# apapiu/transformer_latent_diffusion

Hardware: AMD Instinct MI355X
Metric: images/sec (256px, 35-step CFG sampling), denoiser only (higher is better)
Workload: dtype bf16; 1 GPU; C1: 100M-param denoiser (d=768, L=12), 32x32x4 latents, 35 steps + CFG 6, DPM-Solver++(2M), 64 images/GPU (model batch 128); images_per_gpu=64, global_batch=64, n_iter=35, parallelism=single GPU

## Files before the change

### transformer_latent_diffusion_amd/_lib.py

```python
from __future__ import annotations

import ctypes as C
import os

_HERE = os.path.dirname(os.path.abspath(__file__))
LIB_PATH = os.environ.get("TLD_LIB", os.path.join(_HERE, "libtld_hip.so"))

DTYPE_F32, DTYPE_BF16, DTYPE_F16 = 0, 1, 2

KERNEL_CLASSES = ("gemm_qkv", "gemm_up", "gemm_down", "attention", "cross_row", "dwconv_gelu", "layernorm",
                  "embed", "tail", "update", "conditioning")

ABI_SYMBOLS = (
    "tld_engine_create", "tld_engine_load_tensor", "tld_engine_finalize_weights", "tld_denoiser_forward",
    "tld_sample", "tld_sample_from", "tld_engine_set_gemm_dtype", "tld_engine_set_low_latency", "tld_debug_gemm_splitk", "tld_debug_quant_mx8", "tld_debug_quant_mx8_host", "tld_debug_gemm_mx8",
    "tld_engine_set_debug", "tld_engine_read_stage", "tld_engine_stage_shape", "tld_engine_set_debug_step", "tld_engine_debug_paths", "tld_debug_gemm_bf16", "tld_debug_gemm_bench", "tld_debug_gemm_plan", "tld_debug_gemm_epilogue",
    "tld_engine_set_profile", "tld_engine_profile_reserve", "tld_engine_get_profile", "tld_engine_weight_bytes", "tld_engine_destroy",
    "tld_vae_create", "tld_vae_load_tensor", "tld_vae_finalize_weights", "tld_vae_decode", "tld_vae_set_debug",
    "tld_vae_read_stage", "tld_vae_set_profile", "tld_vae_get_profile", "tld_debug_conv3x3", "tld_vae_weight_bytes",
    "tld_vae_destroy",
    "tld_vae_enc_create", "tld_vae_enc_load_tensor", "tld_vae_enc_finalize_weights", "tld_vae_enc_encode", "tld_vae_enc_set_debug",
    "tld_vae_enc_read_stage", "tld_vae_enc_set_profile", "tld_vae_enc_get_profile", "tld_vae_enc_weight_bytes", "tld_vae_enc_destroy",
    "tld_debug_conv3x3_s2",
    "tld_clip_create", "tld_clip_load_tensor", "tld_clip_finalize_weights", "tld_clip_encode_text", "tld_clip_read_buffer", "tld_clip_weight_bytes",
    "tld_clip_destroy",
    "tld_train_create", "tld_train_param_count", "tld_train_tensor_count", "tld_train_param_layout", "tld_train_set_angular_speeds", "tld_train_bind",
# ... 170 lines not shown
```

### transformer_latent_diffusion_amd/csrc/tld_common.h

```cpp
#pragma once
#include <hip/hip_runtime.h>
#include <atomic>
#include <mutex>
#include <stdint.h>
#include "tld_gemm_plan.h"

namespace tld {

typedef __attribute__((ext_vector_type(8))) __bf16 bf16x8;
typedef __attribute__((ext_vector_type(4))) __bf16 bf16x4;
typedef __attribute__((ext_vector_type(2))) __bf16 bf16x2;
typedef __attribute__((ext_vector_type(16))) float f32x16;
typedef __attribute__((ext_vector_type(4))) float f32x4;
typedef __attribute__((ext_vector_type(4))) unsigned u32x4;
typedef __attribute__((ext_vector_type(8))) int i32x8;
typedef __attribute__((ext_vector_type(2))) float f32x2;

constexpr int kWave = 64;
constexpr int kHeadDim = 64;
constexpr float kLnEps = 1e-5f;

template <int CTRL>
__device__ __forceinline__ float dpp_add(float v) {
    const int s = __builtin_amdgcn_update_dpp(0, __float_as_int(v), CTRL, 0xf, 0xf, true);
// ... 314 lines not shown
};
void launch_tail(const TailParams& p, hipStream_t s);

struct UpdateParams {
    const float* x0_2b;
    float* x_t;
    float* x0_prev;
    float* x0_out;
    float* trace_x0; float* trace_xt;
    float g, a, b, c, c1, c2, sharp, bright;
    int final_step;
    int batch, img, chan_stride, C;
};
void launch_update(const UpdateParams& p, hipStream_t s);

struct UpdateFromParams {
    UpdateParams u;
    const float* noise;
    const float* z0;
    const float* mask;
    float s_next;
};
void launch_update_from(const UpdateFromParams& p, hipStream_t s);
void launch_start_mix(const float* noise, const float* z0, float s0, float* x_t, int n, hipStream_t s);

void launch_linear_f32(const float* in, int ldi, const float* W, const float* b, float* out, int ldo,
                       int T, int K, int N, int act, hipStream_t s);
void launch_sinusoid(const float* sigma, const float* angular, float* out, int T, int half, hipStream_t s);
void launch_layernorm_f32(const float* x, const float* g, const float* b, float* out, int M, int d,
                          hipStream_t s);
// ... 12 lines not shown
```

### transformer_latent_diffusion_amd/csrc/tld_engine.hip

```cpp
#include "../../include/tld_hip.h"
#include "tld_common.h"

#include <cmath>
#include <cstdarg>
#include <cstdio>
#include <cstring>
#include <cstdlib>
#include <map>
#include <string>
#include <vector>

using namespace tld;

namespace {

thread_local char g_err[512] = "";

int fail(int code, const char* fmt, ...) {
    va_list ap;
    va_start(ap, fmt);
    vsnprintf(g_err, sizeof(g_err), fmt, ap);
    va_end(ap);
    return code;
}
// ... 50 lines not shown
    float *up_c1 = nullptr, *up_b1 = nullptr;
    float *n1_w = nullptr, *n1_b = nullptr, *n2_w = nullptr, *n2_b = nullptr, *n3_w = nullptr, *n3_b = nullptr;
    float *kv_w = nullptr, *q_w = nullptr;
};

enum { ST_F32 = 0, ST_BF16 = 1, ST_U8 = 2, ST_MX8S = 3, ST_MX8W = 4 };
inline size_t st_bytes(int dtype) { return dtype == ST_F32 ? 4 : dtype == ST_BF16 ? 2 : 1; }
enum { UNPACK_NONE = 0, UNPACK_QKV_ROWS = 1 };
struct DbgStage {
    void* ptr = nullptr; const void* aux = nullptr; int dtype = ST_F32; int64_t shape[4] = {1, 1, 1, 1};
    bool owned = false; size_t cap = 0; bool live = false;
    int64_t outer_stride = 0; int unpack = UNPACK_NONE;
};

enum KClass { KC_GEMM_QKV = 0, KC_GEMM_UP, KC_GEMM_DOWN, KC_ATTN, KC_CROSS, KC_DWCONV, KC_LN, KC_EMBED,
              KC_TAIL, KC_UPDATE, KC_COND, KC_COUNT };

}

struct tld_engine {
    tld_config cfg{};
    int d = 0, L = 0, H = 0, ntok = 0, grid = 0, pd = 0, hid = 0, img = 0, ne = 0, text = 0;
    bool finalized = false;
    bool fuse_dwconv = true;
    bool fp8 = false;
    bool fp8_fused = true;
    uint8_t *a8 = nullptr, *as8 = nullptr;
    std::map<std::string, HostTensor> host;
    std::vector<void*> allocs;
    int64_t weight_bytes = 0;

// ... 3 lines not shown
          *plin_b = nullptr, *pln2_w = nullptr, *pln2_b = nullptr, *pos = nullptr, *out_w = nullptr,
          *out_b = nullptr;
    bf16* out_w_hl = nullptr;
    bf16* plin_w_hl = nullptr;
    std::vector<Layer> layers;
    const float **tab_kv_w = nullptr, **tab_q_w = nullptr, **tab_n2_w = nullptr, **tab_n2_b = nullptr;

    resid_t* x = nullptr;
    resid_t* x_half = nullptr;
    bool share_l0 = true;
    bool fold_ln1 = true;
    bool low_latency = false;
    float* splitk = nullptr;
    int ll_split = 0;
    bool fuse_qkv_attn = true;
    float2* ln_stats = nullptr;
    bool fold_ln3 = true;
    float2* row_stats = nullptr;
    bf16 *xn = nullptr, *qk = nullptr, *vt = nullptr, *att = nullptr, *hid1 = nullptr, *hid2 = nullptr;
    uint32_t* seam = nullptr;
    float *io_x = nullptr, *io_sigma = nullptr, *io_label = nullptr, *io_out = nullptr;
    float *xt = nullptr, *x0_prev = nullptr, *x0_cfg = nullptr;
    int* rows_dev = nullptr;
    int64_t rows_cap = 0;
    void* stage_host = nullptr;
    size_t stage_cap = 0;
    hipEvent_t stage_ev = nullptr;

    int cond_cap = 0;
    float *c_sigma = nullptr, *c_sin = nullptr, *c_h1 = nullptr, *c_pre = nullptr, *c_y = nullptr,
// ... 250 lines not shown
                     (size_t)e->cond_cap * e->H * d, e->c_bwq, (size_t)e->cond_cap * e->H, T, e->H, d, e->L, s);
    return TLD_OK;
}

void cond_noise_rows(tld_engine* e, int Tn, hipStream_t s) {
    launch_sinusoid(e->c_sigma, e->angular, e->c_sin, Tn, e->ne / 2, s);
    launch_linear_f32(e->c_sin, e->ne, e->ff1_w, e->ff1_b, e->c_h1, e->d, Tn, e->ne, e->d, 1, s);
    launch_linear_f32(e->c_h1, e->d, e->ff3_w, e->ff3_b, e->c_pre, e->d, Tn, e->d, e->d, 0, s);
}

void cond_label_rows(tld_engine* e, int row0, int Tl, hipStream_t s) {
    launch_linear_f32(e->c_label, e->text, e->label_w, e->label_b, e->c_pre + (size_t)row0 * e->d, e->d, Tl,
                      e->text, e->d, 0, s);
}

int run_body(tld_engine* e, const float* x_src, int src_batch, int batch, const int* noise_row,
             const int* label_row, float* out, hipStream_t s, bool share_l0 = false) {
    const int d = e->d, M = batch * e->ntok;
    share_l0 = share_l0 && e->share_l0 && batch == 2 * src_batch;
    if (int rc = debug_poison(e, s)) return rc;
    const int b0 = share_l0 ? src_batch : batch;
    resid_t* xe = share_l0 ? e->x_half : e->x;
    const bool fold1 = e->fold_ln1;
    const int ln_slots = gemm_resid_stat_slots(d);
    {
        ProfScope ps(e, KC_EMBED, s);
        EmbedParams ep{};
        ep.x = x_src; ep.conv_w = e->conv_w; ep.conv_b = e->conv_b; ep.ln1_w = e->pln1_w; ep.ln1_b = e->pln1_b;
        ep.lin_wt = e->plin_wt; ep.lin_w_hl = e->plin_w_hl; ep.lin_b = e->plin_b; ep.ln2_w = e->pln2_w; ep.ln2_b = e->pln2_b; ep.pos = e->pos;
        ep.tok = xe; ep.stats_out = fold1 ? e->ln_stats : nullptr; ep.batch = b0; ep.src_batch = src_batch; ep.C = e->cfg.n_channels;
        ep.S = e->cfg.image_size; ep.p = e->cfg.patch_size; ep.grid = e->grid; ep.pd = e->pd; ep.d = d;
        ep.ntok = e->ntok;
        launch_embed(ep, s);
    }
    const int rdt = sizeof(resid_t) == 2 ? ST_BF16 : ST_F32;
    SNAP("tokens0", xe, rdt, s, (int64_t)b0 * e->ntok, d);
    for (int l = 0; l < e->L; ++l) {
        const Layer& Ly = e->layers[l];
        const bool half = share_l0 && l == 0;
        const int bl = half ? b0 : batch, Ml = bl * e->ntok;
        const bool fuse8 = e->fp8 && e->fp8_fused;
        SNAP(blk_name(l, "x_in"), half ? xe : e->x, rdt, s, Ml, d);
        if (fold1) SNAP(blk_name(l, "ln1"), e->ln_stats, ST_F32, s, Ml, kLnSlots, 2);
        if (!fold1) {
            ProfScope ps(e, KC_LN, s);
            if (fuse8 && layernorm_mx8_supported(d)) launch_layernorm_mx8(half ? xe : e->x, Ly.n1_w, Ly.n1_b, e->a8, e->as8, Ml, d, s);
            else { launch_layernorm_bf16(half ? xe : e->x, Ly.n1_w, Ly.n1_b, e->xn, Ml, d, s); SNAP(blk_name(l, "xn1"), e->xn, ST_BF16, s, Ml, d); }
        }
// ... 110 lines not shown
            ProfScope ps(e, KC_GEMM_DOWN, s);
            GemmParams g{};
            g.A = e->hid2; g.lda = e->hid; g.W = Ly.down_w; g.ldw = e->hid; g.M = M; g.N = d; g.K = e->hid;
            g.bias = Ly.down_b; g.resid = e->x; g.ldr = d;
            g.stats_out = (fold1 && l + 1 < e->L) ? e->ln_stats : nullptr;
            if (e->fp8) {
                if (!(fuse8 && e->grid > 16)) launch_quant_mx8(e->hid2, e->a8, e->as8, M, e->hid, s);
                SNAP(blk_name(l, "a8_down.q"), e->a8, ST_U8, s, M, e->hid); SNAP(blk_name(l, "a8_down.s"), e->as8, ST_MX8S, s, M, e->hid / 32);
                g.f8 = 1; g.A = reinterpret_cast<const bf16*>(e->a8); g.W = reinterpret_cast<const bf16*>(Ly.down_w8);
                g.a_scale = e->as8; g.w_scale = Ly.down_s8;
            }
            launch_gemm(g, EPI_BIAS_RESID, s);
        }
        SNAP(blk_name(l, "mlp"), e->x, rdt, s, M, d);
    }
    {
        ProfScope ps(e, KC_TAIL, s);
        TailParams tp{};
        tp.tok = e->x; tp.w = e->out_w; tp.w_hl = e->out_w_hl; tp.b = e->out_b; tp.out = out; tp.batch = batch;
        tp.C = e->cfg.n_channels; tp.S = e->cfg.image_size; tp.p = e->cfg.patch_size; tp.grid = e->grid;
        tp.pd = e->pd; tp.d = d; tp.ntok = e->ntok;
        launch_tail(tp, s);
    }
    SNAP("out", out, ST_F32, s, batch, e->img);
    HIP_TRY(hipGetLastError());
    return TLD_OK;
}

int sample_prepare(tld_engine* e, const void* labels, const float* coeffs, int n_levels, int batch, hipStream_t s, const int** label_row_out) {
    if (!e->finalized) return fail(TLD_ERR_STATE, "weights not finalized");
    if (batch <= 0 || 2 * batch > e->cfg.max_batch)
        return fail(TLD_ERR_INVALID, "sampler batch %d needs max_batch >= %d (have %d)", batch, 2 * batch, e->cfg.max_batch);
    if (n_levels < 2) return fail(TLD_ERR_INVALID, "need at least two noise levels");
    const int B = batch, B2 = 2 * batch, T = n_levels + B + 1;
    if (int rc = ensure_cond_capacity(e, T)) return rc;
    if (int rc = ensure_rows_capacity(e, (int64_t)(n_levels + 1) * B2)) return rc;

    const size_t n_rows = (size_t)(n_levels + 1) * B2;
    if (int rc = debug_begin(e, T, n_levels, s)) return rc;
// ... 22 lines not shown

UpdateParams update_params(tld_engine* e, const float* coeffs, int n_levels, int i, float class_guidance, float sharp_f, float bright_f,
                           void* out_latent, int B, void* trace_x0, void* trace_xt) {
    const bool final_step = (i == n_levels - 1);
    const size_t tot = (size_t)B * e->img;
    UpdateParams up{};
    const float* c = coeffs + (size_t)i * 6;
    up.x0_2b = e->io_out; up.x_t = e->xt; up.x0_prev = e->x0_prev;
    up.x0_out = final_step ? static_cast<float*>(out_latent) : e->x0_cfg;
    up.trace_x0 = (!final_step && trace_x0) ? static_cast<float*>(trace_x0) + (size_t)i * tot : nullptr;
    up.trace_xt = (!final_step && trace_xt) ? static_cast<float*>(trace_xt) + (size_t)i * tot : nullptr;
    up.g = class_guidance; up.a = c[1]; up.b = c[2]; up.c = c[3]; up.c1 = c[4]; up.c2 = c[5];
    up.sharp = sharp_f; up.bright = bright_f; up.final_step = final_step ? 1 : 0;
    up.batch = B; up.img = e->img; up.chan_stride = e->cfg.image_size * e->cfg.image_size; up.C = e->cfg.n_channels;
    return up;
}

int step_begin(tld_engine* e, int i, int B, hipStream_t s) {
    e->dbg_keep = e->debug && (e->dbg_step < 0 || e->dbg_step == i);
    SNAP("step.x_t", e->xt, ST_F32, s, B, e->img); SNAP("step.x0_prev", e->x0_prev, ST_F32, s, B, e->img);
    return TLD_OK;
}
int step_end(tld_engine* e, const UpdateParams& up, int B, hipStream_t s) {
    SNAP("step.out", e->io_out, ST_F32, s, 2 * B, e->img); SNAP("step.x0", up.x0_out, ST_F32, s, B, e->img);
    if (!up.final_step) SNAP("step.x_next", e->xt, ST_F32, s, B, e->img);
    e->dbg_keep = false;
    return TLD_OK;
}

}
// ... 43 lines not shown
    hipDeviceProp_t prop;
    HIP_TRY(hipGetDeviceProperties(&prop, c->device_id));
    if (strncmp(prop.gcnArchName, "gfx950", 6) != 0)
        return fail(TLD_ERR_INVALID, "device %d is %s; this engine is built for gfx950 only", c->device_id, prop.gcnArchName);
    tld_engine* e = new tld_engine();
    e->cfg = *c;
    e->d = c->embed_dim; e->L = c->n_layers; e->H = c->embed_dim / 64; e->grid = grid; e->ntok = ntok;
    e->pd = pd; e->hid = c->mlp_multiplier * c->embed_dim; e->img = c->n_channels * c->image_size * c->image_size;
    e->ne = c->noise_embed_dims; e->text = c->text_emb_size;
    e->layers.resize(e->L);
    if (const char* fd = getenv("TLD_FUSE_DWCONV")) e->fuse_dwconv = atoi(fd) != 0;
    if (const char* sl = getenv("TLD_SHARE_L0")) e->share_l0 = atoi(sl) != 0;
    if (const char* f8 = getenv("TLD_FP8_FUSED")) e->fp8_fused = atoi(f8) != 0;
    if (const char* fl = getenv("TLD_FOLD_LN3")) e->fold_ln3 = atoi(fl) != 0;
    if (const char* fl = getenv("TLD_FOLD_LN1")) e->fold_ln1 = atoi(fl) != 0;
#ifndef TLD_RESID_BF16
    e->fold_ln3 = false;
    e->fold_ln1 = false;
#endif
    e->fold_ln1 = e->fold_ln1 && gemm_resid_stat_slots(e->d) > 0 && (3 * e->d) % 256 == 0;
    e->fold_ln3 = e->fold_ln3 && e->hid % 256 == 0 && cross_row_supports_ln3_stats(e->d);
    if (const char* fq = getenv("TLD_FUSE_QKV_ATTN")) e->fuse_qkv_attn = atoi(fq) != 0;
    e->fuse_qkv_attn = e->fuse_qkv_attn && e->fold_ln1 && ntok == 256 && e->d % 128 == 0;
    *out = e;
    return TLD_OK;
}

int tld_engine_load_tensor(tld_engine* e, const char* key, const void* host_ptr, const int64_t* shape,
                           int32_t ndim, int32_t dtype) {
    if (!e || !key || (!host_ptr && ndim > 0)) return fail(TLD_ERR_INVALID, "null argument");
// ... 416 lines not shown
int tld_sample(tld_engine* e, const void* x_T, const void* labels, const float* coeffs, int32_t n_levels,
               float class_guidance, float sharp_f, float bright_f, void* out_latent, int32_t batch,
               void* trace_x0, void* trace_xt, void* hip_stream) {
    if (!e || !x_T || !labels || !coeffs || !out_latent) return fail(TLD_ERR_INVALID, "null argument");
    DeviceGuard dg(e->cfg.device_id);
    hipStream_t s = static_cast<hipStream_t>(hip_stream);
    const int* label_row = nullptr;
    PathScope paths(e);
    if (int rc = sample_prepare(e, labels, coeffs, n_levels, batch, s, &label_row)) return rc;
    const int B = batch, B2 = 2 * batch;

    const size_t tot = (size_t)B * e->img;
    HIP_TRY(hipMemcpyAsync(e->xt, x_T, tot * sizeof(float), hipMemcpyDeviceToDevice, s));
    HIP_TRY(hipMemsetAsync(e->x0_prev, 0, tot * sizeof(float), s));

    for (int i = 0; i < n_levels; ++i) {
        if (int rc = step_begin(e, i, B, s)) return rc;
        if (int rc = run_body(e, e->xt, B, B2, e->rows_dev + (size_t)i * B2, label_row, e->io_out, s, true)) return rc;
        const UpdateParams up = update_params(e, coeffs, n_levels, i, class_guidance, sharp_f, bright_f, out_latent, B, trace_x0, trace_xt);
        {
            ProfScope ps(e, KC_UPDATE, s);
            launch_update(up, s);
        }
        if (int rc = step_end(e, up, B, s)) return rc;
    }
    HIP_TRY(hipGetLastError());
    return TLD_OK;
}

int tld_sample_from(tld_engine* e, const void* noise, const void* init_latent, const void* mask, float start_mix, const void* labels,
                    const float* coeffs, int32_t n_levels, float class_guidance, float sharp_f, float bright_f, void* out_latent,
// ... 1 lines not shown
    if (!e || !noise || !labels || !coeffs || !out_latent) return fail(TLD_ERR_INVALID, "null argument");
    if (!(start_mix > 0.0f && start_mix <= 1.0f)) return fail(TLD_ERR_INVALID, "start_mix %g outside (0, 1]", (double)start_mix);
    if (!init_latent && (mask || start_mix < 1.0f)) return fail(TLD_ERR_INVALID, "init_latent is required with a mask or with start_mix < 1");
    DeviceGuard dg(e->cfg.device_id);
    hipStream_t s = static_cast<hipStream_t>(hip_stream);
    const int* label_row = nullptr;
    PathScope paths(e);
    if (int rc = sample_prepare(e, labels, coeffs, n_levels, batch, s, &label_row)) return rc;
    const int B = batch, B2 = 2 * batch;

    const size_t tot = (size_t)B * e->img;
    if (start_mix == 1.0f) HIP_TRY(hipMemcpyAsync(e->xt, noise, tot * sizeof(float), hipMemcpyDeviceToDevice, s));
    else launch_start_mix(static_cast<const float*>(noise), static_cast<const float*>(init_latent), start_mix, e->xt, (int)tot, s);
    HIP_TRY(hipMemsetAsync(e->x0_prev, 0, tot * sizeof(float), s));

    for (int i = 0; i < n_levels; ++i) {
        if (int rc = step_begin(e, i, B, s)) return rc;
        if (int rc = run_body(e, e->xt, B, B2, e->rows_dev + (size_t)i * B2, label_row, e->io_out, s, true)) return rc;
        UpdateFromParams uf{};
        uf.u = update_params(e, coeffs, n_levels, i, class_guidance, sharp_f, bright_f, out_latent, B, trace_x0, trace_xt);
        uf.noise = static_cast<const float*>(noise); uf.z0 = static_cast<const float*>(init_latent); uf.mask = static_cast<const float*>(mask);
        uf.s_next = (i + 1 < n_levels) ? coeffs[(size_t)(i + 1) * 6 + 0] : 0.0f;
        {
            ProfScope ps(e, KC_UPDATE, s);
            launch_update_from(uf, s);
        }
        if (int rc = step_end(e, uf.u, B, s)) return rc;
    }
    HIP_TRY(hipGetLastError());
    return TLD_OK;
}
// ... 309 lines not shown
```

### transformer_latent_diffusion_amd/csrc/tld_rows.hip

```cpp
#include "tld_common.h"
#include <cstdlib>

namespace tld {

namespace {


template <int NJ, bool HALF>
__global__ __launch_bounds__(256) void embed_kernel(EmbedParams p) {
    extern __shared__ __attribute__((aligned(16))) char smem[];
    constexpr int d = NJ * 128 - (HALF ? 64 : 0);
    float* wt = reinterpret_cast<float*>(smem);
    float* cwt = wt + p.pd * d;
    for (int i = threadIdx.x; i < p.pd * d / 4; i += 256)
        reinterpret_cast<float4*>(wt)[i] = reinterpret_cast<const float4*>(p.lin_wt)[i];
    for (int i = threadIdx.x; i < p.pd * p.C * p.p * p.p; i += 256) {
        const int o = i / (p.C * p.p * p.p), k = i - o * (p.C * p.p * p.p);
        cwt[k * p.pd + o] = p.conv_w[i];
    }
    __syncthreads();
    const int lane = threadIdx.x & 63;
    const int wid = __builtin_amdgcn_readfirstlane(threadIdx.x >> 6);
    const bool live_last = !HALF || lane < 32;
    auto live = [&](int j) { return j + 1 < NJ || live_last; };
// ... 645 lines not shown
            const int u = uv / p.p, vv = uv - u * p.p;
#pragma unroll
            for (int u2 = 0; u2 < 2; ++u2) {
                const int r = row + u2;
                if (r < total) {
                    const int b = r / p.ntok, t = r - b * p.ntok;
                    const int ti = t / p.grid, tj = t - ti * p.grid;
                    p.out[(((size_t)b * p.C + c) * p.S + (ti * p.p + u)) * p.S + (tj * p.p + vv)] = mine[u2];
                }
            }
        }
    }
}

#ifdef TLD_RESID_BF16
template <int TPW>
__global__ __launch_bounds__(256) void embed_mfma_kernel(EmbedParams p, const bf16* __restrict__ wl_hl) {
    extern __shared__ __attribute__((aligned(16))) char smem[];
    constexpr int d = TPW * 128, PD = 16, PP = 144;
    float* cw = reinterpret_cast<float*>(smem);
    float* red = cw + PD * PD;
    float* vec = red + 4 * 4 * 32;
    char* patch = reinterpret_cast<char*>(vec + 3 * d);
    const int lane = threadIdx.x & 63;
    const int wid = __builtin_amdgcn_readfirstlane(threadIdx.x >> 6);
    const int l31 = lane & 31, hi = lane >> 5;
    const int total = p.batch * p.ntok;
    const int grow = blockIdx.x * 32 + l31;
    const int row = grow < total ? grow : total - 1;
    const int b = row / p.ntok, tk = row - b * p.ntok;
    const int ti = tk / p.grid, tj = tk - ti * p.grid;
    float xin[PD];
    {
        const int pp = p.p * p.p;
        const float* xb = p.x + (size_t)(b % p.src_batch) * p.C * p.S * p.S;
#pragma unroll
        for (int k = 0; k < PD; ++k) {
            const int c = k / pp, uv = k - c * pp, u = uv / p.p, v = uv - u * p.p;
            xin[k] = xb[((size_t)c * p.S + (ti * p.p + u)) * p.S + (tj * p.p + v)];
        }
    }
    bf16x8 whf[TPW], wlf[TPW];
#pragma unroll
    for (int t = 0; t < TPW; ++t) {
        const int f = 32 * (wid * TPW + t) + l31;
        whf[t] = *reinterpret_cast<const bf16x8*>(wl_hl + (size_t)f * PD + hi * 8);
        wlf[t] = *reinterpret_cast<const bf16x8*>(wl_hl + ((size_t)d + f) * PD + hi * 8);
    }
    if (threadIdx.x < PD * PD) cw[threadIdx.x] = p.conv_w[threadIdx.x];
    for (int i = threadIdx.x; i < 3 * d / 4; i += 256) {
        const int which = i / (d / 4), j = i - which * (d / 4);
        const float* src = which == 0 ? p.lin_b : (which == 1 ? p.ln2_w : p.ln2_b);
        reinterpret_cast<float4*>(vec)[i] = reinterpret_cast<const float4*>(src)[j];
    }
    __syncthreads();
    float pv[8];
// ... 106 lines not shown
        }
        __builtin_amdgcn_fence(__ATOMIC_ACQUIRE, "wavefront");
    }
    if (p.stats_out) {
        ssum = pair_sum(ssum); ssq = pair_sum(ssq);
        if (!hi) { red[256 + wid * 32 + l31] = ssum; red[384 + wid * 32 + l31] = ssq; }
        __syncthreads();
        if (wid == 0 && !hi && grow < total) {
            const float a = (red[256 + l31] + red[288 + l31]) + (red[320 + l31] + red[352 + l31]);
            const float a2 = (red[384 + l31] + red[416 + l31]) + (red[448 + l31] + red[480 + l31]);
            *reinterpret_cast<float4*>(p.stats_out + (size_t)grow * kLnSlots) = make_float4(a, a2, 0.f, 0.f);
        }
    }
}

template <int NT>
__global__ __launch_bounds__(256) void tail_mfma_kernel(TailParams p, const bf16* __restrict__ whl) {
    extern __shared__ __attribute__((aligned(16))) char smem[];
    const int d = p.d, PITCH = d * 2, pdp = NT * 16;
    char* wh = smem;
    char* wl = smem + pdp * PITCH;
    const int chunks = d >> 3;
    for (int i = threadIdx.x; i < 2 * pdp * chunks; i += 256) {
        const int plane = i / (pdp * chunks), rem = i - plane * pdp * chunks;
        const int r = rem / chunks, c = rem - r * chunks;
        u32x4 v = {0u, 0u, 0u, 0u};
        if (r < p.pd) v = *reinterpret_cast<const u32x4*>(whl + ((size_t)plane * p.pd + r) * d + c * 8);
        *reinterpret_cast<u32x4*>((plane ? wl : wh) + r * PITCH + ((c ^ (r & 15)) << 4)) = v;
    }
    __syncthreads();
    const int lane = threadIdx.x & 63, wid = threadIdx.x >> 6;
    const int tok = lane & 15, kq = lane >> 4;
    const int total = p.batch * p.ntok;
    const int row0 = (blockIdx.x * 4 + wid) * 16;
    if (row0 >= total) return;
    const int row = row0 + tok < total ? row0 + tok : total - 1;
    const bf16* xrow = p.tok + (size_t)row * d + kq * 8;
    f32x4 acc[NT];
#pragma unroll
    for (int t = 0; t < NT; ++t) acc[t] = f32x4{0.f, 0.f, 0.f, 0.f};
    const int nkb = d >> 5;
    constexpr int PF = 8;
    bf16x8 xf[PF];
#pragma unroll
    for (int i = 0; i < PF; ++i) xf[i] = *reinterpret_cast<const bf16x8*>(xrow + (i < nkb ? i : 0) * 32);
    for (int kb0 = 0; kb0 < nkb; kb0 += PF) {
#pragma unroll
        for (int i = 0; i < PF; ++i) {
            const int kb = kb0 + i;
            if (kb >= nkb) break;
            const bf16x8 xb = xf[i];
            if (kb + PF < nkb) xf[i] = *reinterpret_cast<const bf16x8*>(xrow + (kb + PF) * 32);
            const int chunk = 4 * kb + kq;
#pragma unroll
            for (int t = 0; t < NT; ++t) {
                const int r = t * 16 + tok;
                const int off = r * PITCH + ((chunk ^ (r & 15)) << 4);
                acc[t] = __builtin_amdgcn_mfma_f32_16x16x32_bf16(*reinterpret_cast<const bf16x8*>(wh + off), xb, acc[t], 0, 0, 0);
                acc[t] = __builtin_amdgcn_mfma_f32_16x16x32_bf16(*reinterpret_cast<const bf16x8*>(wl + off), xb, acc[t], 0, 0, 0);
            }
        }
    }
    if (row0 + tok >= total) return;
    const int b = row / p.ntok, tk = row - b * p.ntok;
    const int ti = tk / p.grid, tj = tk - ti * p.grid;
    const int pp = p.p * p.p;
#pragma unroll
    for (int t = 0; t < NT; ++t)
#pragma unroll
        for (int r = 0; r < 4; ++r) {
            const int f = t * 16 + 4 * kq + r;
            if (f < p.pd) {
                const int c = f / pp, uv = f - c * pp;
                const int u = uv / p.p, vv = uv - u * p.p;
                p.out[(((size_t)b * p.C + c) * p.S + (ti * p.p + u)) * p.S + (tj * p.p + vv)] = acc[t][r] + p.b[f];
            }
        }
// ... 82 lines not shown

template <int V>
__global__ __launch_bounds__(256) void start_mix_kernel(const float* __restrict__ noise, const float* __restrict__ z0, float s0,
                                                        float* __restrict__ x_t, int n) {
#pragma clang fp contract(off)
    const int i = (blockIdx.x * 256 + threadIdx.x) * V;
    if (i >= n) return;
    if constexpr (V == 4) {
        const float4 e = *reinterpret_cast<const float4*>(noise + i), z = *reinterpret_cast<const float4*>(z0 + i);
        const float t = 1.0f - s0;
        *reinterpret_cast<float4*>(x_t + i) = make_float4(s0 * e.x + t * z.x, s0 * e.y + t * z.y, s0 * e.z + t * z.z, s0 * e.w + t * z.w);
    } else {
        x_t[i] = s0 * noise[i] + (1.0f - s0) * z0[i];
    }
}

constexpr int DW_CB = 64;
__global__ __launch_bounds__(256) void dwconv_gelu_kernel(const bf16* __restrict__ in, bf16* __restrict__ out,
                                                          const float* __restrict__ w9c,
                                                          const float* __restrict__ bias, int batch,
                                                          int g, int C) {
    extern __shared__ __attribute__((aligned(16))) char smem[];
    const int nchunk = C / DW_CB;
    const int b = blockIdx.x / nchunk, cc = blockIdx.x - b * nchunk;
    const int ntok = g * g;
    const bf16* src = in + (size_t)b * ntok * C + cc * DW_CB;
    for (int idx = threadIdx.x; idx < ntok * 8; idx += 256) {
        const int t = idx >> 3, q = idx & 7;
        *reinterpret_cast<uint4*>(smem + t * 128 + q * 16) =
            *reinterpret_cast<const uint4*>(src + (size_t)t * C + q * 8);
// ... 187 lines not shown
    do {                                                                                             \
        if ((dd) % 128) TLD_DISPATCH_NJ_(((dd) + 127) / 128, true, __VA_ARGS__) else TLD_DISPATCH_NJ_((dd) / 128, false, __VA_ARGS__)  \
    } while (0)

#define TLD_LDS_OPT_IN(KERNEL, bytes)                                                                \
    do {                                                                                             \
        static PerDeviceMax optin;                                                                   \
        if ((bytes) > 64 * 1024)                                                                     \
            optin.run((bytes), [&] { hipFuncSetAttribute(reinterpret_cast<const void*>(KERNEL), hipFuncAttributeMaxDynamicSharedMemorySize, (bytes)); }); \
    } while (0)

void launch_embed(const EmbedParams& p, hipStream_t s) {
#ifdef TLD_RESID_BF16
    if (p.lin_w_hl && p.pd == 16 && p.C * p.p * p.p == 16 && p.d % 256 == 0 && p.d <= 1024) {
        const int rows = p.batch * p.ntok;
        const int lds = 16 * 16 * 4 + 4 * 4 * 32 * 4 + 3 * p.d * 4 + 4 * 32 * 144;
        dim3 grid((unsigned)((rows + 31) / 32));
#define TLD_EM(TPW) do { TLD_LDS_OPT_IN((embed_mfma_kernel<TPW>), lds); hipLaunchKernelGGL((embed_mfma_kernel<TPW>), grid, dim3(256), lds, s, p, p.lin_w_hl); } while (0)
        note_path(EP_EMBED_MFMA + p.d / 256 - 1);
        if (p.d == 256) TLD_EM(2); else if (p.d == 512) TLD_EM(4); else if (p.d == 768) TLD_EM(6); else TLD_EM(8);
#undef TLD_EM
        return;
    }
#endif
    const int rows = p.batch * p.ntok;
    const int lds = (p.pd * p.d + p.pd * p.C * p.p * p.p) * (int)sizeof(float);
    note_path(EP_EMBED_PLAIN);
    TLD_DISPATCH_D(p.d, { TLD_LDS_OPT_IN((embed_kernel<NJ, HALF>), lds); hipLaunchKernelGGL((embed_kernel<NJ, HALF>), dim3((rows + 31) / 32), dim3(256), lds, s, p); });
}

void launch_layernorm_bf16(const resid_t* x, const float* g, const float* b, bf16* out, int M, int d,
// ... 110 lines not shown
#undef TLD_TM
        return;
    }
#endif
    const int rpb = 64;
    const int rows = p.batch * p.ntok;
    const int lds = p.pd * p.d * (int)sizeof(float);
    note_path(EP_TAIL_PLAIN);
    TLD_DISPATCH_D(p.d, { TLD_LDS_OPT_IN((tail_kernel<NJ, HALF>), lds); hipLaunchKernelGGL((tail_kernel<NJ, HALF>), dim3((rows + rpb - 1) / rpb), dim3(256), lds, s, p, rpb); });
}

void launch_update(const UpdateParams& p, hipStream_t s) {
    const int n = p.batch * p.img;
    note_path(EP_UPDATE);
    hipLaunchKernelGGL(update_kernel, dim3((n + 255) / 256), dim3(256), 0, s, p);
}

namespace {
bool aligned16(const void* a) { return (reinterpret_cast<uintptr_t>(a) & 15) == 0; }
}

void launch_update_from(const UpdateFromParams& q, hipStream_t s) {
    const UpdateParams& p = q.u;
    const int n = p.batch * p.img;
    const bool vec = p.img % 4 == 0 && p.chan_stride % 4 == 0 && aligned16(p.x0_2b) && aligned16(p.x_t) && aligned16(p.x0_prev) && aligned16(p.x0_out) &&
                     aligned16(p.trace_x0) && aligned16(p.trace_xt) && aligned16(q.noise) && aligned16(q.z0) && aligned16(q.mask);
    const int threads = vec ? n / 4 : n;
    const dim3 grid((threads + 255) / 256), block(256);
    note_path(q.mask ? EP_UPDATE_FROM_MASK : EP_UPDATE_FROM);
    if (q.mask) {
// ... 242 lines not shown
```

Baseline: 295.3 images/s.

## Fuse tail projection, solver update and next-step embed into one boundary kernel

Adds a step_boundary kernel that, between denoiser steps, does the output projection for both CFG streams, applies the DPM-Solver update, and immediately re-embeds the new latent for the next step. The whole boundary runs per 32-token tile in LDS, replacing three launches and their global round-trips. Also drops the separate step_begin path when fused. The path only runs when share_l0 is on, with no mask, debug, profiling or fp8. It risks numerical differences from the reordered solver arithmetic and higher LDS use per block.

```diff
diff --git a/transformer_latent_diffusion_amd/_lib.py b/transformer_latent_diffusion_amd/_lib.py
--- a/transformer_latent_diffusion_amd/_lib.py
+++ b/transformer_latent_diffusion_amd/_lib.py
@@ -9,7 +9,7 @@
 DTYPE_F32, DTYPE_BF16, DTYPE_F16 = 0, 1, 2
 
 KERNEL_CLASSES = ("gemm_qkv", "gemm_up", "gemm_down", "attention", "cross_row", "dwconv_gelu", "layernorm",
-                  "embed", "tail", "update", "conditioning")
+                  "embed", "tail", "update", "conditioning", "boundary")
 
 ABI_SYMBOLS = (
     "tld_engine_create", "tld_engine_load_tensor", "tld_engine_finalize_weights", "tld_denoiser_forward",
diff --git a/transformer_latent_diffusion_amd/csrc/tld_common.h b/transformer_latent_diffusion_amd/csrc/tld_common.h
--- a/transformer_latent_diffusion_amd/csrc/tld_common.h
+++ b/transformer_latent_diffusion_amd/csrc/tld_common.h
@@ -352,6 +352,10 @@
 };
 void launch_update(const UpdateParams& p, hipStream_t s);
 
+struct BoundaryParams { TailParams t; UpdateParams u; EmbedParams e; };
+bool step_boundary_supported(int d, int pd, int C, int p);
+void launch_step_boundary(const BoundaryParams& q, hipStream_t s);
+
 struct UpdateFromParams {
     UpdateParams u;
     const float* noise;
diff --git a/transformer_latent_diffusion_amd/csrc/tld_engine.hip b/transformer_latent_diffusion_amd/csrc/tld_engine.hip
--- a/transformer_latent_diffusion_amd/csrc/tld_engine.hip
+++ b/transformer_latent_diffusion_amd/csrc/tld_engine.hip
@@ -88,7 +88,7 @@
 };
 
 enum KClass { KC_GEMM_QKV = 0, KC_GEMM_UP, KC_GEMM_DOWN, KC_ATTN, KC_CROSS, KC_DWCONV, KC_LN, KC_EMBED,
-              KC_TAIL, KC_UPDATE, KC_COND, KC_COUNT };
+              KC_TAIL, KC_UPDATE, KC_COND, KC_BOUNDARY, KC_COUNT };
 
 }
 
@@ -122,6 +122,7 @@
     float* splitk = nullptr;
     int ll_split = 0;
     bool fuse_qkv_attn = true;
+    bool fuse_boundary = true;
     float2* ln_stats = nullptr;
     bool fold_ln3 = true;
     float2* row_stats = nullptr;
@@ -402,8 +403,27 @@
                       e->text, e->d, 0, s);
 }
 
+EmbedParams embed_params(const tld_engine* e, const float* x_src, int src_batch, int batch, resid_t* tok) {
+    EmbedParams ep{};
+    ep.x = x_src; ep.conv_w = e->conv_w; ep.conv_b = e->conv_b; ep.ln1_w = e->pln1_w; ep.ln1_b = e->pln1_b;
+    ep.lin_wt = e->plin_wt; ep.lin_w_hl = e->plin_w_hl; ep.lin_b = e->plin_b; ep.ln2_w = e->pln2_w; ep.ln2_b = e->pln2_b; ep.pos = e->pos;
+    ep.tok = tok; ep.stats_out = e->fold_ln1 ? e->ln_stats : nullptr; ep.batch = batch; ep.src_batch = src_batch; ep.C = e->cfg.n_channels;
+    ep.S = e->cfg.image_size; ep.p = e->cfg.patch_size; ep.grid = e->grid; ep.pd = e->pd; ep.d = e->d;
+    ep.ntok = e->ntok;
+    return ep;
+}
+TailParams tail_params(const tld_engine* e, float* out, int batch) {
+    TailParams tp{};
+    tp.tok = e->x; tp.w = e->out_w; tp.w_hl = e->out_w_hl; tp.b = e->out_b; tp.out = out; tp.batch = batch;
+    tp.C = e->cfg.n_channels; tp.S = e->cfg.image_size; tp.p = e->cfg.patch_size; tp.grid = e->grid;
+    tp.pd = e->pd; tp.d = e->d; tp.ntok = e->ntok;
+    return tp;
+}
+
+enum { BODY_EMBED = 1, BODY_TAIL = 2, BODY_ALL = 3 };
+
 int run_body(tld_engine* e, const float* x_src, int src_batch, int batch, const int* noise_row,
-             const int* label_row, float* out, hipStream_t s, bool share_l0 = false) {
+             const int* label_row, float* out, hipStream_t s, bool share_l0 = false, int parts = BODY_ALL) {
     const int d = e->d, M = batch * e->ntok;
     share_l0 = share_l0 && e->share_l0 && batch == 2 * src_batch;
     if (int rc = debug_poison(e, s)) return rc;
@@ -411,15 +431,9 @@
     resid_t* xe = share_l0 ? e->x_half : e->x;
     const bool fold1 = e->fold_ln1;
     const int ln_slots = gemm_resid_stat_slots(d);
-    {
+    if (parts & BODY_EMBED) {
         ProfScope ps(e, KC_EMBED, s);
-        EmbedParams ep{};
-        ep.x = x_src; ep.conv_w = e->conv_w; ep.conv_b = e->conv_b; ep.ln1_w = e->pln1_w; ep.ln1_b = e->pln1_b;
-        ep.lin_wt = e->plin_wt; ep.lin_w_hl = e->plin_w_hl; ep.lin_b = e->plin_b; ep.ln2_w = e->pln2_w; ep.ln2_b = e->pln2_b; ep.pos = e->pos;
-        ep.tok = xe; ep.stats_out = fold1 ? e->ln_stats : nullptr; ep.batch = b0; ep.src_batch = src_batch; ep.C = e->cfg.n_channels;
-        ep.S = e->cfg.image_size; ep.p = e->cfg.patch_size; ep.grid = e->grid; ep.pd = e->pd; ep.d = d;
-        ep.ntok = e->ntok;
-        launch_embed(ep, s);
+        launch_embed(embed_params(e, x_src, src_batch, b0, xe), s);
     }
     const int rdt = sizeof(resid_t) == 2 ? ST_BF16 : ST_F32;
     SNAP("tokens0", xe, rdt, s, (int64_t)b0 * e->ntok, d);
@@ -560,15 +574,13 @@
         }
         SNAP(blk_name(l, "mlp"), e->x, rdt, s, M, d);
     }
-    {
-        ProfScope ps(e, KC_TAIL, s);
-        TailParams tp{};
-        tp.tok = e->x; tp.w = e->out_w; tp.w_hl = e->out_w_hl; tp.b = e->out_b; tp.out = out; tp.batch = batch;
-        tp.C = e->cfg.n_channels; tp.S = e->cfg.image_size; tp.p = e->cfg.patch_size; tp.grid = e->grid;
-        tp.pd = e->pd; tp.d = d; tp.ntok = e->ntok;
-        launch_tail(tp, s);
-    }
-    SNAP("out", out, ST_F32, s, batch, e->img);
+    if (parts & BODY_TAIL) {
+        {
+            ProfScope ps(e, KC_TAIL, s);
+            launch_tail(tail_params(e, out, batch), s);
+        }
+        SNAP("out", out, ST_F32, s, batch, e->img);
+    }
     HIP_TRY(hipGetLastError());
     return TLD_OK;
 }
@@ -621,6 +633,28 @@
     up.sharp = sharp_f; up.bright = bright_f; up.final_step = final_step ? 1 : 0;
     up.batch = B; up.img = e->img; up.chan_stride = e->cfg.image_size * e->cfg.image_size; up.C = e->cfg.n_channels;
     return up;
+}
+
+bool boundary_fused(const tld_engine* e, bool masked) {
+    const uint32_t replaced = (1u << KC_EMBED) | (1u << KC_TAIL) | (1u << KC_UPDATE);
+    return e->fuse_boundary && e->share_l0 && !masked && !e->debug && !(e->prof_mask & replaced) && !e->fp8 && e->out_w_hl && e->plin_w_hl &&
+           step_boundary_supported(e->d, e->pd, e->cfg.n_channels, e->cfg.patch_size);
+}
+
+int fused_step(tld_engine* e, const UpdateParams& up, int i, int B, const int* noise_row, const int* label_row, hipStream_t s) {
+    const int parts = (i == 0 ? BODY_EMBED : 0) | (up.final_step ? BODY_TAIL : 0);
+    if (int rc = run_body(e, e->xt, B, 2 * B, noise_row, label_row, e->io_out, s, true, parts)) return rc;
+    if (up.final_step) {
+        ProfScope ps(e, KC_UPDATE, s);
+        launch_update(up, s);
+    } else {
+        ProfScope ps(e, KC_BOUNDARY, s);
+        BoundaryParams bp{};
+        bp.t = tail_params(e, nullptr, 2 * B); bp.u = up; bp.e = embed_params(e, nullptr, B, B, e->x_half);
+        launch_step_boundary(bp, s);
+    }
+    HIP_TRY(hipGetLastError());
+    return TLD_OK;
 }
 
 int step_begin(tld_engine* e, int i, int B, hipStream_t s) {
@@ -694,6 +728,7 @@
     if (const char* f8 = getenv("TLD_FP8_FUSED")) e->fp8_fused = atoi(f8) != 0;
     if (const char* fl = getenv("TLD_FOLD_LN3")) e->fold_ln3 = atoi(fl) != 0;
     if (const char* fl = getenv("TLD_FOLD_LN1")) e->fold_ln1 = atoi(fl) != 0;
+    if (const char* fb = getenv("TLD_FUSE_BOUNDARY")) e->fuse_boundary = atoi(fb) != 0;
 #ifndef TLD_RESID_BF16
     e->fold_ln3 = false;
     e->fold_ln1 = false;
@@ -1140,7 +1175,13 @@
     HIP_TRY(hipMemcpyAsync(e->xt, x_T, tot * sizeof(float), hipMemcpyDeviceToDevice, s));
     HIP_TRY(hipMemsetAsync(e->x0_prev, 0, tot * sizeof(float), s));
 
+    const bool fused = boundary_fused(e, false);
     for (int i = 0; i < n_levels; ++i) {
+        if (fused) {
+            const UpdateParams up = update_params(e, coeffs, n_levels, i, class_guidance, sharp_f, bright_f, out_latent, B, trace_x0, trace_xt);
+            if (int rc = fused_step(e, up, i, B, e->rows_dev + (size_t)i * B2, label_row, s)) return rc;
+            continue;
+        }
         if (int rc = step_begin(e, i, B, s)) return rc;
         if (int rc = run_body(e, e->xt, B, B2, e->rows_dev + (size_t)i * B2, label_row, e->io_out, s, true)) return rc;
         const UpdateParams up = update_params(e, coeffs, n_levels, i, class_guidance, sharp_f, bright_f, out_latent, B, trace_x0, trace_xt);
@@ -1172,7 +1213,13 @@
     else launch_start_mix(static_cast<const float*>(noise), static_cast<const float*>(init_latent), start_mix, e->xt, (int)tot, s);
     HIP_TRY(hipMemsetAsync(e->x0_prev, 0, tot * sizeof(float), s));
 
+    const bool fused = boundary_fused(e, mask != nullptr);
     for (int i = 0; i < n_levels; ++i) {
+        if (fused) {
+            const UpdateParams up = update_params(e, coeffs, n_levels, i, class_guidance, sharp_f, bright_f, out_latent, B, trace_x0, trace_xt);
+            if (int rc = fused_step(e, up, i, B, e->rows_dev + (size_t)i * B2, label_row, s)) return rc;
+            continue;
+        }
         if (int rc = step_begin(e, i, B, s)) return rc;
         if (int rc = run_body(e, e->xt, B, B2, e->rows_dev + (size_t)i * B2, label_row, e->io_out, s, true)) return rc;
         UpdateFromParams uf{};
diff --git a/transformer_latent_diffusion_amd/csrc/tld_rows.hip b/transformer_latent_diffusion_amd/csrc/tld_rows.hip
--- a/transformer_latent_diffusion_amd/csrc/tld_rows.hip
+++ b/transformer_latent_diffusion_amd/csrc/tld_rows.hip
@@ -683,9 +683,9 @@
 }
 
 #ifdef TLD_RESID_BF16
+constexpr int kEmbedMfmaLdsFixed = 16 * 16 * 4 + 4 * 4 * 32 * 4 + 4 * 32 * 144;
 template <int TPW>
-__global__ __launch_bounds__(256) void embed_mfma_kernel(EmbedParams p, const bf16* __restrict__ wl_hl) {
-    extern __shared__ __attribute__((aligned(16))) char smem[];
+__device__ __forceinline__ void embed_rows_mfma(const EmbedParams& p, const bf16* __restrict__ wl_hl, char* smem, const float (&xin)[16], int tk) {
     constexpr int d = TPW * 128, PD = 16, PP = 144;
     float* cw = reinterpret_cast<float*>(smem);
     float* red = cw + PD * PD;
@@ -696,19 +696,6 @@
     const int l31 = lane & 31, hi = lane >> 5;
     const int total = p.batch * p.ntok;
     const int grow = blockIdx.x * 32 + l31;
-    const int row = grow < total ? grow : total - 1;
-    const int b = row / p.ntok, tk = row - b * p.ntok;
-    const int ti = tk / p.grid, tj = tk - ti * p.grid;
-    float xin[PD];
-    {
-        const int pp = p.p * p.p;
-        const float* xb = p.x + (size_t)(b % p.src_batch) * p.C * p.S * p.S;
-#pragma unroll
-        for (int k = 0; k < PD; ++k) {
-            const int c = k / pp, uv = k - c * pp, u = uv / p.p, v = uv - u * p.p;
-            xin[k] = xb[((size_t)c * p.S + (ti * p.p + u)) * p.S + (tj * p.p + v)];
-        }
-    }
     bf16x8 whf[TPW], wlf[TPW];
 #pragma unroll
     for (int t = 0; t < TPW; ++t) {
@@ -845,20 +832,78 @@
     }
 }
 
-template <int NT>
-__global__ __launch_bounds__(256) void tail_mfma_kernel(TailParams p, const bf16* __restrict__ whl) {
+template <int TPW>
+__global__ __launch_bounds__(256) void embed_mfma_kernel(EmbedParams p, const bf16* __restrict__ wl_hl) {
     extern __shared__ __attribute__((aligned(16))) char smem[];
-    const int d = p.d, PITCH = d * 2, pdp = NT * 16;
+    constexpr int PD = 16;
+    const int l31 = threadIdx.x & 31;
+    const int total = p.batch * p.ntok;
+    const int grow = blockIdx.x * 32 + l31;
+    const int row = grow < total ? grow : total - 1;
+    const int b = row / p.ntok, tk = row - b * p.ntok;
+    const int ti = tk / p.grid, tj = tk - ti * p.grid;
+    float xin[PD];
+    {
+        const int pp = p.p * p.p;
+        const float* xb = p.x + (size_t)(b % p.src_batch) * p.C * p.S * p.S;
+#pragma unroll
+        for (int k = 0; k < PD; ++k) {
+            const int c = k / pp, uv = k - c * pp, u = uv / p.p, v = uv - u * p.p;
+            xin[k] = xb[((size_t)c * p.S + (ti * p.p + u)) * p.S + (tj * p.p + v)];
+        }
+    }
+    embed_rows_mfma<TPW>(p, wl_hl, smem, xin, tk);
+}
+
+__device__ __forceinline__ void tail_fill_weights(char* smem, const bf16* __restrict__ whl, int pd, int pdp, int d) {
+    const int PITCH = d * 2, chunks = d >> 3;
     char* wh = smem;
     char* wl = smem + pdp * PITCH;
-    const int chunks = d >> 3;
     for (int i = threadIdx.x; i < 2 * pdp * chunks; i += 256) {
         const int plane = i / (pdp * chunks), rem = i - plane * pdp * chunks;
         const int r = rem / chunks, c = rem - r * chunks;
         u32x4 v = {0u, 0u, 0u, 0u};
-        if (r < p.pd) v = *reinterpret_cast<const u32x4*>(whl + ((size_t)plane * p.pd + r) * d + c * 8);
+        if (r < pd) v = *reinterpret_cast<const u32x4*>(whl + ((size_t)plane * pd + r) * d + c * 8);
         *reinterpret_cast<u32x4*>((plane ? wl : wh) + r * PITCH + ((c ^ (r & 15)) << 4)) = v;
     }
+}
+
+template <int NT>
+__device__ __forceinline__ void tail_rows_mfma(const char* smem, const bf16* __restrict__ xrow, int d, int tok, int kq, f32x4 (&acc)[NT]) {
+    const int PITCH = d * 2, pdp = NT * 16;
+    const char* wh = smem;
+    const char* wl = smem + pdp * PITCH;
+#pragma unroll
+    for (int t = 0; t < NT; ++t) acc[t] = f32x4{0.f, 0.f, 0.f, 0.f};
+    const int nkb = d >> 5;
+    constexpr int PF = 8;
+    bf16x8 xf[PF];
+#pragma unroll
+    for (int i = 0; i < PF; ++i) xf[i] = *reinterpret_cast<const bf16x8*>(xrow + (i < nkb ? i : 0) * 32);
+    for (int kb0 = 0; kb0 < nkb; kb0 += PF) {
+#pragma unroll
+        for (int i = 0; i < PF; ++i) {
+            const int kb = kb0 + i;
+            if (kb >= nkb) break;
+            const bf16x8 xb = xf[i];
+            if (kb + PF < nkb) xf[i] = *reinterpret_cast<const bf16x8*>(xrow + (kb + PF) * 32);
+            const int chunk = 4 * kb + kq;
+#pragma unroll
+            for (int t = 0; t < NT; ++t) {
+                const int r = t * 16 + tok;
+                const int off = r * PITCH + ((chunk ^ (r & 15)) << 4);
+                acc[t] = __builtin_amdgcn_mfma_f32_16x16x32_bf16(*reinterpret_cast<const bf16x8*>(wh + off), xb, acc[t], 0, 0, 0);
+                acc[t] = __builtin_amdgcn_mfma_f32_16x16x32_bf16(*reinterpret_cast<const bf16x8*>(wl + off), xb, acc[t], 0, 0, 0);
+            }
+        }
+    }
+}
+
+template <int NT>
+__global__ __launch_bounds__(256) void tail_mfma_kernel(TailParams p, const bf16* __restrict__ whl) {
+    extern __shared__ __attribute__((aligned(16))) char smem[];
+    const int d = p.d;
+    tail_fill_weights(smem, whl, p.pd, NT * 16, d);
     __syncthreads();
     const int lane = threadIdx.x & 63, wid = threadIdx.x >> 6;
     const int tok = lane & 15, kq = lane >> 4;
@@ -866,32 +911,8 @@
     const int row0 = (blockIdx.x * 4 + wid) * 16;
     if (row0 >= total) return;
     const int row = row0 + tok < total ? row0 + tok : total - 1;
-    const bf16* xrow = p.tok + (size_t)row * d + kq * 8;
     f32x4 acc[NT];
-#pragma unroll
-    for (int t = 0; t < NT; ++t) acc[t] = f32x4{0.f, 0.f, 0.f, 0.f};
-    const int nkb = d >> 5;
-    constexpr int PF = 8;
-    bf16x8 xf[PF];
-#pragma unroll
-    for (int i = 0; i < PF; ++i) xf[i] = *reinterpret_cast<const bf16x8*>(xrow + (i < nkb ? i : 0) * 32);
-    for (int kb0 = 0; kb0 < nkb; kb0 += PF) {
-#pragma unroll
-        for (int i = 0; i < PF; ++i) {
-            const int kb = kb0 + i;
-            if (kb >= nkb) break;
-            const bf16x8 xb = xf[i];
-            if (kb + PF < nkb) xf[i] = *reinterpret_cast<const bf16x8*>(xrow + (kb + PF) * 32);
-            const int chunk = 4 * kb + kq;
-#pragma unroll
-            for (int t = 0; t < NT; ++t) {
-                const int r = t * 16 + tok;
-                const int off = r * PITCH + ((chunk ^ (r & 15)) << 4);
-                acc[t] = __builtin_amdgcn_mfma_f32_16x16x32_bf16(*reinterpret_cast<const bf16x8*>(wh + off), xb, acc[t], 0, 0, 0);
-                acc[t] = __builtin_amdgcn_mfma_f32_16x16x32_bf16(*reinterpret_cast<const bf16x8*>(wl + off), xb, acc[t], 0, 0, 0);
-            }
-        }
-    }
+    tail_rows_mfma<NT>(smem, p.tok + (size_t)row * d + kq * 8, d, tok, kq, acc);
     if (row0 + tok >= total) return;
     const int b = row / p.ntok, tk = row - b * p.ntok;
     const int ti = tk / p.grid, tj = tk - ti * p.grid;
@@ -1004,6 +1025,79 @@
         x_t[i] = s0 * noise[i] + (1.0f - s0) * z0[i];
     }
 }
+
+#ifdef TLD_RESID_BF16
+__device__ __forceinline__ void solver_update(const UpdateParams& p, float cond, float unc, float prev, float xin, float& x0, float& xt) {
+#pragma clang fp contract(off)
+    x0 = __builtin_fmaf(p.g, cond, (1.0f - p.g) * unc);
+    const float D = __builtin_fmaf(p.c1, x0, -(p.c2 * prev));
+    xt = (p.a * D + p.b * xin) / p.c;
+}
+
+template <int TPW>
+__global__ __launch_bounds__(256) void step_boundary_kernel(BoundaryParams q) {
+    extern __shared__ __attribute__((aligned(16))) char smem[];
+    constexpr int d = TPW * 128, PD = 16;
+    constexpr int region = 2 * 16 * d * 2 > kEmbedMfmaLdsFixed + 3 * d * 4 ? 2 * 16 * d * 2 : kEmbedMfmaLdsFixed + 3 * d * 4;
+    float* pred = reinterpret_cast<float*>(smem + region);
+    float* xnew = pred + 2 * 32 * PD;
+    const EmbedParams& ep = q.e;
+    const int B = ep.batch, ntok = ep.ntok, total = B * ntok;
+    const int lane = threadIdx.x & 63, wid = threadIdx.x >> 6;
+    tail_fill_weights(smem, q.t.w_hl, PD, 16, d);
+    __syncthreads();
+    {
+        const int tok = lane & 15, kq = lane >> 4;
+        const int stream = wid >> 1, lt = 16 * (wid & 1) + tok;
+        const int grow = blockIdx.x * 32 + lt;
+        const int row = grow < total ? grow : total - 1;
+        f32x4 acc[1];
+        tail_rows_mfma<1>(smem, q.t.tok + ((size_t)stream * total + row) * d + kq * 8, d, tok, kq, acc);
+#pragma unroll
+        for (int r = 0; r < 4; ++r) acc[0][r] = acc[0][r] + q.t.b[4 * kq + r];
+        *reinterpret_cast<f32x4*>(pred + (stream * 32 + lt) * PD + 4 * kq) = acc[0];
+    }
+    __syncthreads();
+    {
+        const UpdateParams& up = q.u;
+        const int lt = threadIdx.x >> 3, f0 = 2 * (threadIdx.x & 7);
+        const int grow = blockIdx.x * 32 + lt;
+        if (grow < total) {
+            const int b = grow / ntok, tk = grow - b * ntok;
+            const int ti = tk / ep.grid, tj = tk - ti * ep.grid;
+            const int pp = ep.p * ep.p;
+#pragma unroll
+            for (int e = 0; e < 2; ++e) {
+                const int f = f0 + e;
+                const int c = f / pp, uv = f - c * pp, u = uv / ep.p, vv = uv - u * ep.p;
+                const size_t i = (((size_t)b * ep.C + c) * ep.S + (ti * ep.p + u)) * ep.S + (tj * ep.p + vv);
+                float x0, xt;
+                solver_update(up, pred[lt * PD + f], pred[(32 + lt) * PD + f], up.x0_prev[i], up.x_t[i], x0, xt);
+                up.x0_out[i] = x0;
+                if (up.trace_x0) up.trace_x0[i] = x0;
+                up.x_t[i] = xt;
+                up.x0_prev[i] = x0;
+                if (up.trace_xt) up.trace_xt[i] = xt;
+                xnew[lt * PD + f] = xt;
+            }
+        } else {
+            xnew[lt * PD + f0] = 0.f; xnew[lt * PD + f0 + 1] = 0.f;
+        }
+    }
+    __syncthreads();
+    const int l31 = lane & 31;
+    const int grow = blockIdx.x * 32 + l31;
+    const int row = grow < total ? grow : total - 1;
+    const int src = row - blockIdx.x * 32;
+    float xin[PD];
+#pragma unroll
+    for (int k4 = 0; k4 < PD / 4; ++k4) {
+        const float4 t = *reinterpret_cast<const float4*>(xnew + src * PD + 4 * k4);
+        xin[4 * k4] = t.x; xin[4 * k4 + 1] = t.y; xin[4 * k4 + 2] = t.z; xin[4 * k4 + 3] = t.w;
+    }
+    embed_rows_mfma<TPW>(ep, ep.lin_w_hl, smem, xin, row % ntok);
+}
+#endif
 
 constexpr int DW_CB = 64;
 __global__ __launch_bounds__(256) void dwconv_gelu_kernel(const bf16* __restrict__ in, bf16* __restrict__ out,
@@ -1221,7 +1315,7 @@
 #ifdef TLD_RESID_BF16
     if (p.lin_w_hl && p.pd == 16 && p.C * p.p * p.p == 16 && p.d % 256 == 0 && p.d <= 1024) {
         const int rows = p.batch * p.ntok;
-        const int lds = 16 * 16 * 4 + 4 * 4 * 32 * 4 + 3 * p.d * 4 + 4 * 32 * 144;
+        const int lds = kEmbedMfmaLdsFixed + 3 * p.d * 4;
         dim3 grid((unsigned)((rows + 31) / 32));
 #define TLD_EM(TPW) do { TLD_LDS_OPT_IN((embed_mfma_kernel<TPW>), lds); hipLaunchKernelGGL((embed_mfma_kernel<TPW>), grid, dim3(256), lds, s, p, p.lin_w_hl); } while (0)
         note_path(EP_EMBED_MFMA + p.d / 256 - 1);
@@ -1362,6 +1456,26 @@
     const int n = p.batch * p.img;
     note_path(EP_UPDATE);
     hipLaunchKernelGGL(update_kernel, dim3((n + 255) / 256), dim3(256), 0, s, p);
+}
+
+bool step_boundary_supported(int d, int pd, int C, int p) {
+#ifdef TLD_RESID_BF16
+    return pd == 16 && C * p * p == 16 && d % 256 == 0 && d <= 1024;
+#else
+    return false;
+#endif
+}
+
+void launch_step_boundary(const BoundaryParams& q, hipStream_t s) {
+#ifdef TLD_RESID_BF16
+    const int d = q.e.d, rows = q.e.batch * q.e.ntok;
+    const int region = 2 * 16 * d * 2 > kEmbedMfmaLdsFixed + 3 * d * 4 ? 2 * 16 * d * 2 : kEmbedMfmaLdsFixed + 3 * d * 4;
+    const int lds = region + 3 * 32 * 16 * 4;
+    dim3 grid((unsigned)((rows + 31) / 32));
+#define TLD_SB(TPW) do { TLD_LDS_OPT_IN((step_boundary_kernel<TPW>), lds); hipLaunchKernelGGL((step_boundary_kernel<TPW>), grid, dim3(256), lds, s, q); } while (0)
+    if (d == 256) TLD_SB(2); else if (d == 512) TLD_SB(4); else if (d == 768) TLD_SB(6); else TLD_SB(8);
+#undef TLD_SB
+#endif
 }
 
 namespace {
```

Result: no change. 295.2 images/s (median of 2 runs) (-0.0%).
